# malani86/unet-DC-segmentation

Hardware: AMD Instinct MI355X
Metric: images/sec fwd+bwd, 512x512x1 U-Net-DC, bs=8/GPU (higher is better)
Workload: dtype bf16

## Files before the change

quantify_droplets_batch.py:

```python
#!/usr/bin/env python3
import argparse
import dataclasses
from pathlib import Path

import numpy as np
import pandas as pd
import torch
from PIL import Image

from models.model_2 import UNetDC
from unet_dc_segmentation_amd.droplets import DropletOptions, Droplets, resize_mask_like_reference
from utils import intensity_window as iw
from utils.data_loader import resize_image, rolling_ball_correction_rgb

DEVICE = "cuda" if torch.cuda.is_available() else "cpu"
IMG_SIZE = 512


def load_model(ckpt, dtype="f32"):
    m = UNetDC(in_channels=3, out_channels=1)
    m.load_state_dict(torch.load(ckpt, map_location=DEVICE, weights_only=True))
    m.set_compute_dtype(dtype)
    return m.to(DEVICE).eval()

# ... 763 lines not shown
        raise SystemExit("--boundary measures against annotated masks: it needs --gt_dir")
    from utils.droplet_boundary import DEFAULT_TOLS, check_radius, check_tols
    try:
        R = check_radius(args.boundary)
        tols = DEFAULT_TOLS if args.boundary_tol is None else [int(v) for v in args.boundary_tol.split(",") if v.strip()]
        tols = check_tols([t for t in tols if args.boundary_tol is not None or t <= R], R)
    except ValueError as e:
        raise SystemExit(f"--boundary R / --boundary_tol: {e}")
    return {"R": R, "tols": tols, "records": []}


def confidence_options(args):
    if args.confidence is None:
        if args.confidence_maps:
            raise SystemExit("--confidence_maps needs --confidence")
        return None
    from utils.droplet_confidence import check_band
    try:
        band = check_band(args.confidence)
    except ValueError as e:
        raise SystemExit(f"--confidence BAND: {e}")
    return {"band": band, "maps": bool(args.confidence_maps), "rows": []}


def spatial_options(args, images):
    if args.spatial_stats is None:
        if args.spatial_window_dir:
            raise SystemExit("--spatial_window_dir belongs to --spatial_stats")
        return None
    from utils.spatial_stats import check_sims
    try:
        sims = check_sims(args.spatial_sims)
    except ValueError as e:
        raise SystemExit(f"--spatial_sims S: {e}")
    if not 0 <= args.spatial_seed < 2 ** 32:
        raise SystemExit("--spatial_seed must be in 0..2^32 - 1")
    files = None
    if args.spatial_window_dir:
        files = find_gt_files(images, args.spatial_window_dir, "--spatial_window_dir", "window")
    return {"R": args.spatial_stats, "S": sims, "seed": args.spatial_seed, "files": files, "table": [], "rows": []}


def tile_options(args):
    if args.tile is None:
        if args.tile_overlap is not None:
            raise SystemExit("--tile_overlap needs --tile")
        return None
    from utils.tiling import check_tile
    try:
        T, O = check_tile(args.tile, 64 if args.tile_overlap is None else args.tile_overlap)
    except ValueError as e:
        raise SystemExit(f"--tile / --tile_overlap: {e}")
    if args.batch < 1:
        raise SystemExit("--tile: --batch is the number of tiles per forward, at least 1")
    return {"T": T, "O": O}


def tta_options(args):
    if args.tta is None:
        return None
    from utils.tta import TTA_SIZES
    if args.tta not in TTA_SIZES:
        raise SystemExit(f"--tta N: N must be one of {', '.join(map(str, TTA_SIZES))}, not {args.tta}")
    if args.batch < 1:
        raise SystemExit("--tta: --batch is the number of items per forward, at least 1")
    return None if args.tta == 1 else {"N": args.tta, "batch": args.batch}


def main(argv=None):
    parser = build_parser()
    args = parser.parse_args(argv)
    if args.gt_dir and args.gt_polygons:
        parser.error("--gt_polygons and --gt_dir are two sources of the same annotation: give one")
    if args.diff_maps is not None and not (args.gt_dir or args.gt_polygons):
        parser.error("--diff_maps compares against annotated masks: it needs --gt_dir")
    if args.diff_maps is not None and args.diff_maps < 1:
        parser.error("--diff_maps MIN_AREA: MIN_AREA is a number of pixels, at least 1")
    in_dir, out_dir = Path(args.img_dir), Path(args.out_dir)
    try:
        spec = iw.spec_from_flags(args.intensity_window, args.intensity_levels, args.page)
    except ValueError as e:
        parser.error(str(e))
    intensity = None if spec is None else {"spec": spec, "records": []}
    iw.clip_warner.done = False
    from utils.droplet_split import half_pixels
    try:
        split_depth = half_pixels(args.split_depth) / 2.0
    except ValueError:
        raise SystemExit("--split_depth must be a non-negative multiple of 0.5")
    if not args.split_touching:
        split_depth = None
    clean = clean_options(args)
    sweep = sweep_options(args)
    tile = tile_options(args)
    tta = tta_options(args)
    boundary = boundary_options(args)
    confidence = confidence_options(args)
    hull = None
    if args.droplet_hull is not None:
        from utils.droplet_hull import check_solidity
        try:
            hull = check_solidity(args.droplet_hull)
        except ValueError as e:
            raise SystemExit(f"--droplet_hull S: {e}")
    images = sorted(p for p in in_dir.iterdir() if p.suffix.lower() in IMAGE_SUFFIXES)
    gt = None
    if args.gt_dir:
        gt = {"files": find_gt_files(images, args.gt_dir), "min_area": args.gt_min_area, "labels": args.gt_labels}
    elif args.gt_polygons:
        gt = {"polygons": find_gt_polygons(images, args.gt_polygons), "min_area": 1, "labels": True, "features": 0, "dropped": 0}
    spatial = spatial_options(args, images)
    mask_dir = out_dir / "predicted_masks"
    overlay_dir = out_dir / "overlays" if args.save_overlays else None
    out_dir.mkdir(parents=True, exist_ok=True)
    mask_dir.mkdir(exist_ok=True)
    if overlay_dir:
        overlay_dir.mkdir(exist_ok=True)
    density = None
    if args.density_maps:
        if not 1 <= args.nb_layers <= 255 or not 0 < args.density_kernel or int(4 * args.density_kernel / 6 + 0.5) > 128:
            raise SystemExit("--nb_layers must be in 1..255 and --density_kernel in 1..192")
        density = {"nb_layers": args.nb_layers, "kernel": args.density_kernel}
    diff = None
    if args.diff_maps is not None:
        diff = {"min_area": args.diff_maps, "map_dir": out_dir / "difference_maps", "overlay_dir": out_dir / "diff_overlays",
                "tables": [], "rows": []}
        diff["map_dir"].mkdir(exist_ok=True)
        diff["overlay_dir"].mkdir(exist_ok=True)
    outlines = None
    if args.outlines:
        outlines = {"dir": out_dir / "outlines", "images": [], "jobs": []}
        outlines["dir"].mkdir(exist_ok=True)
    model = load_model(args.ckpt_path, args.dtype)
    import os
    from collections import deque
    from concurrent.futures import ThreadPoolExecutor
    nthreads = max(1, min(8, (os.cpu_count() or 2) // 2))
    with ThreadPoolExecutor(nthreads) as dec_pool, ThreadPoolExecutor(nthreads) as wr_pool:
        run = Run(thresh=args.prob_thresh, min_area=args.min_area, px_per_um=args.px_per_micron,
                  background_radius=args.background_radius, batch_size=args.batch, split_depth=split_depth,
                  shape=args.droplet_shape, clean=clean, sweep=sweep, tile=tile, tta=tta, density=density, gt=gt, out_dir=out_dir,
                  mask_dir=mask_dir, overlay_dir=overlay_dir, writers=(wr_pool, deque(), 4 * max(1, args.batch)),
                  neighbors=args.neighbors, boundary=boundary, confidence=confidence, hull=hull, diff=diff,
                  spatial=spatial, outlines=outlines, intensity=intensity)
        ahead = deque()
        it = iter(images)

        def refill():
            while len(ahead) < 2 * args.batch:
                nxt = next(it, None)
                if nxt is None:
                    return
                ahead.append((nxt, dec_pool.submit(decode_image, nxt, intensity),
                              None if gt is None else dec_pool.submit(decode_gt_polygons, gt["polygons"][str(nxt)]) if "polygons" in gt
                              else dec_pool.submit(decode_gt, gt["files"][str(nxt)], gt["labels"]),
                              None if spatial is None or spatial["files"] is None
                              else dec_pool.submit(decode_gt, spatial["files"][str(nxt)], False)))

        refill()
        batch = Batch()
        while ahead:
            img, fut, gt_fut, win_fut = ahead.popleft()
            refill()
            im = fut.result()
            if intensity is not None:
                im = window_image(run, img, *im)
            batch.meta.append((str(img), tuple(int(v) for v in im.shape[:2])))
            if run.shape:
                from utils.density import rgb_to_gray
                batch.grays.append(rgb_to_gray(_host(im)))
            if gt is not None:
                batch.gt_items.append(gt_fut.result())
            if win_fut is not None:
                batch.windows.append(win_fut.result())
            if tile is not None:
                probs, rgb = predict_tiled_image(model, _host(im), run)
                batch.rgbs.append(rgb)
                finish_batch(run, batch, probs)
                batch = Batch()
                continue
            t, _, *rgb = preprocess(img, args.background_radius, im, keep_rgb=run.keep_rgb)
            batch.tensors.append(t)
            batch.rgbs += rgb
            if len(batch.tensors) == args.batch:
                run_batch(run, batch, model)
                batch = Batch()
        if batch.tensors:
            run_batch(run, batch, model)
        for f in run.writers[1]:
            f.result()
    if intensity is not None:
        rows = [iw.record_row(name, mode, spec, n, {k: _host(v) for k, v in rec.items()}) for name, mode, n, rec in intensity["records"]]
        pd.DataFrame(rows).to_csv(out_dir / "intensity_per_image.csv", index=False)
    if density is not None:
        pd.DataFrame(run.density_rows).to_csv(out_dir / "density_per_image.csv", index=False)
    if gt is not None:
        from utils.droplet_match import pooled_row, summary_row
        tables = [t for t in run.gt_tables if len(t)] or run.gt_tables[:1]
        pd.concat(tables, ignore_index=True).to_csv(out_dir / "gt_droplets.csv", index=False) if tables else None
        rows = [summary_row(name, ints) for name, ints in run.gt_images] + [pooled_row([ints for _, ints in run.gt_images])]
        pd.DataFrame(rows).to_csv(out_dir / "match_per_image.csv", index=False)
        if "polygons" in gt:
            print(f"--gt_polygons: {gt['dropped']} of {gt['features']} features own no pixel centre and were dropped")
    if boundary is not None:
        from utils import droplet_boundary as db
        recs = boundary["records"]
        rows = [db.summary_row(name, h, d, boundary["R"], boundary["tols"]) for name, h, d in recs]
        rows.append(db.pooled_row([(h, d) for _, h, d in recs], boundary["R"], boundary["tols"]))
        pd.DataFrame(rows, columns=db.column_names(boundary["tols"])).to_csv(out_dir / "boundary_per_image.csv", index=False)
    if confidence is not None:
        from utils.droplet_confidence import IMAGE_COLUMNS
        pd.DataFrame(confidence["rows"], columns=("filename",) + IMAGE_COLUMNS).to_csv(out_dir / "confidence_per_image.csv", index=False)
    if diff is not None:
        from utils import difference_map as dmap
        tables = [t for t in diff["tables"] if len(t)] or diff["tables"][:1]
        pd.concat(tables, ignore_index=True).to_csv(out_dir / "diff_regions.csv", index=False) if tables else None
        pd.DataFrame(diff["rows"], columns=("filename",) + dmap.IMAGE_COLUMNS).to_csv(out_dir / "diff_regions_per_image.csv", index=False)
    if spatial is not None:
        from utils import spatial_stats as ss
        pd.DataFrame(spatial["table"], columns=ss.table_columns(run.px_per_um)).to_csv(out_dir / "spatial_stats.csv", index=False)
        pd.DataFrame(spatial["rows"], columns=ss.IMAGE_COLUMNS).to_csv(out_dir / "spatial_per_image.csv", index=False)
    if outlines is not None:
        import json
        anns = [a for job in outlines["jobs"] for a in job.result()]
        for i, a in enumerate(anns, start=1):
            a["id"] = i
        with open(out_dir / "outlines_coco.json", "w") as f:
            f.write(json.dumps({"images": outlines["images"], "annotations": anns, "categories": [{"id": 1, "name": "droplet"}]},
                               separators=(",", ":")))
    if clean is not None:
        pd.DataFrame(clean["rows"]).to_csv(out_dir / "mask_clean_per_image.csv", index=False)
    if run.neighbors is not None and run.contact_tables:
        pd.concat(run.contact_tables, ignore_index=True).to_csv(out_dir / "droplet_contacts.csv", index=False)
    if sweep is not None and sweep["hist"] is not None:
        from utils.threshold_sweep import summary_line, table_rows
        hist = sweep["hist"]
        if torch.is_tensor(hist):
            from unet_dc_segmentation_amd.evaluate import sweep_result
            hist = sweep_result(hist)
        pd.DataFrame(table_rows(hist)).to_csv(out_dir / "threshold_sweep.csv", index=False)
        print(summary_line(hist))
        if sweep["objects"]:
            from utils.droplet_match import pooled_row
            rows = []
            for t in sweep["objects"]:
                row = pooled_row(sweep["object_images"][t])
                row.pop("filename")
                rows.append({"threshold": t, **row})
            pd.DataFrame(rows).to_csv(out_dir / "threshold_sweep_objects.csv", index=False)
    summary_df = pd.DataFrame(run.rows)
    summary_df.to_csv(out_dir / "summary_per_image.csv", index=False)
    props = [d for d in run.tables if not d.empty]
    if props:
        combined = pd.concat(props, ignore_index=True)
        combined.to_csv(out_dir / "all_droplets.csv", index=False)
        if not args.skip_excel:
            try:
                import xlsxwriter
                with pd.ExcelWriter(out_dir / "all_droplets.xlsx", engine="xlsxwriter") as xw:
                    combined.to_excel(xw, index=False, sheet_name="droplets")
                    summary_df.to_excel(xw, index=False, sheet_name="per_image")
            except (ImportError, AttributeError):
                combined.to_csv(out_dir / "all_droplets_noexcel.csv", index=False)
                print("Skipped Excel file (xlsxwriter not available); wrote all_droplets_noexcel.csv")
        size_col = "eq_diam_micron" if "eq_diam_micron" in combined.columns else "equivalent_diameter"
        stats = combined[size_col].describe()[["mean", "50%", "std"]].rename({"50%": "median"})
        stats.to_csv(out_dir / "droplet_size_stats.csv")
        if not args.skip_histogram:
            import matplotlib
            matplotlib.use("Agg")
            import matplotlib.pyplot as plt
            plt.figure(figsize=(6, 4))
            plt.hist(combined[size_col], bins=40)
# ... 13 lines not shown
```

unet_dc_segmentation_amd/build.py:

```python
from __future__ import annotations

import os
import shutil
import subprocess
import sys

HERE = os.path.dirname(os.path.abspath(__file__))
CSRC = os.path.join(HERE, "csrc")
SOURCES = ["abi.hip", "igemm_conv.hip", "igemm_dma.hip", "igemm_dma16.hip", "igemm_halo.hip", "igemm_lattice.hip", "wgrad.hip", "wgrad_dma.hip", "wgrad_fused.hip", "wgrad_rect.hip", "convt_wgrad.hip", "first_conv.hip", "first_conv_mfma.hip", "partials.hip", "batchnorm.hip", "head.hip", "pack.hip", "loss.hip", "optim.hip", "ccl.hip", "split.hip", "shape.hip", "confidence.hip", "hull.hip", "outlines.hip", "polyfill.hip", "match.hip", "neighbors.hip", "spatial.hip", "boundary.hip", "diffmap.hip", "clean.hip", "sweep.hip", "tile.hip", "tta.hip", "preprocess.hip", "window.hip", "augment.hip", "crop.hip", "density.hip", "border.hip"]
HEADERS = ["common.h", "kernels.h", "workspace.h", "partials.h", "bn_bwd_terms.h", "ccl_uf.h", "pair_table.h", "wave_ops.h", "lds_dma.h", "wgrad_frag.h", "igemm_epilogue.h", "igemm_epilogue16.h", "gather_index.h", "linear_u8.h", "hash32.h", os.path.join("..", "..", "include", "unetdc_hip.h")]
OUT = os.path.join(HERE, "libunetdc_hip.so")


def _hipcc():
    for cand in (shutil.which("hipcc"), "/opt/rocm/bin/hipcc"):
        if cand and os.path.exists(cand):
            return cand
    raise RuntimeError("hipcc not found (ROCm toolchain required to build the gfx950 kernels)")


def needs_build():
    if not os.path.exists(OUT):
        return True
    t = os.path.getmtime(OUT)
    deps = [os.path.join(CSRC, f) for f in SOURCES + HEADERS]
    return any(os.path.getmtime(d) > t for d in deps)


FLAGS = ["--offload-arch=gfx950", "-O3", "-std=c++17", "-fPIC", "-Wall", "-Wno-unused-function", "-fno-slp-vectorize"]
OBJ_DIR = os.path.join(CSRC, "_obj")


def _includes(path, seen=None):
    import re
    seen = set() if seen is None else seen
    for m in re.finditer(r'^\s*#include\s+"([^"]+)"', open(path).read(), re.M):
        q = os.path.normpath(os.path.join(os.path.dirname(path), m.group(1)))
        if q not in seen and os.path.exists(q):
            seen.add(q)
            _includes(q, seen)
    return seen


def _object_key(src):
    import hashlib
    h = hashlib.sha256(" ".join(FLAGS).encode())
    for q in [src] + sorted(_includes(src)):
        h.update(open(q, "rb").read())
    return h.hexdigest()[:16]


def build(force=False, verbose=True):
    if not force and not needs_build():
        return OUT
    from concurrent.futures import ThreadPoolExecutor
    os.makedirs(OBJ_DIR, exist_ok=True)
    hipcc = _hipcc()

    def one(f):
        src = os.path.join(CSRC, f)
        obj = os.path.join(OBJ_DIR, f"{os.path.splitext(f)[0]}.{_object_key(src)}.o")
        if force or not os.path.exists(obj):
            for old in os.listdir(OBJ_DIR):
                if old.startswith(os.path.splitext(f)[0] + "."):
                    os.unlink(os.path.join(OBJ_DIR, old))
            cmd = [hipcc, *FLAGS, "-c", src, "-o", obj]
            if verbose:
                print("[unetdc build]", " ".join(cmd), flush=True)
            r = subprocess.run(cmd, capture_output=True, text=True)
            if r.returncode != 0:
                sys.stderr.write(r.stdout + r.stderr)
                raise RuntimeError(f"hipcc failed on {f}")
        return obj

    with ThreadPoolExecutor(max_workers=min(8, os.cpu_count() or 1)) as ex:
        objs = list(ex.map(one, SOURCES))
    cmd = [hipcc, "--offload-arch=gfx950", "-shared", "-fPIC", *objs, "-o", OUT]
    r = subprocess.run(cmd, capture_output=True, text=True)
    if r.returncode != 0:
        sys.stderr.write(r.stdout + r.stderr)
        raise RuntimeError("hipcc failed linking libunetdc_hip.so")
    return OUT


def _objdump():
    for cand in (shutil.which("llvm-objdump"), "/opt/rocm/lib/llvm/bin/llvm-objdump"):
        if cand and os.path.exists(cand):
            return cand
    raise RuntimeError("llvm-objdump not found")


def device_code_objects(so_path=OUT):
# ... 44 lines not shown
```

unet_dc_segmentation_amd/csrc/igemm_conv.hip:

```cpp
#include <stdlib.h>

#include <stdio.h>

#include "kernels.h"

namespace unetdc {

template <typename T> struct Mma;
template <> struct Mma<bf16_t> {
  __device__ static __forceinline__ void run(f32x16& acc, const u32x4& a, const u32x4& b) {
    acc = __builtin_amdgcn_mfma_f32_32x32x16_bf16(__builtin_bit_cast(bf16x8, a), __builtin_bit_cast(bf16x8, b),
                                                  acc, 0, 0, 0);
  }
};
template <> struct Mma<float> {
  __device__ static __forceinline__ void run(f32x16& acc, const u32x4& a, const u32x4& b) {
#pragma unroll
    for (int s = 0; s < 4; ++s) {
      const unsigned int ua = a[s], ub = b[s];
      acc = __builtin_amdgcn_mfma_f32_32x32x2f32(bits_f32(ua), bits_f32(ub), acc, 0, 0, 0);
    }
  }
};

// ... 180 lines not shown
        store_pair<T>(og + (long)m * p.ldo + col, v0, v1);
        if (p.mode == MODE_STATS) {
          const float t0 = round_through<T>(v0), t1 = round_through<T>(v1);
          s0 += t0; q0 = fmaf(t0, t0, q0);
          s1 += t1; q1 = fmaf(t1, t1, q1);
        }
      }
    }
  }
  if (p.mode == MODE_STATS) {
    s0 += __shfl_xor(s0, 32, 64); q0 += __shfl_xor(q0, 32, 64);
    s1 += __shfl_xor(s1, 32, 64); q1 += __shfl_xor(q1, 32, 64);
    float* red = reinterpret_cast<float*>(smem);
    if (h == 0) {
      red[(wave * 4 + 0) * 32 + r] = s0;
      red[(wave * 4 + 1) * 32 + r] = q0;
      red[(wave * 4 + 2) * 32 + r] = s1;
      red[(wave * 4 + 3) * 32 + r] = q1;
    }
    __syncthreads();
    if (tid < BN) {
      const int wn2 = tid >> 6, c2 = tid & 63, r2 = c2 >> 1, e = c2 & 1;
      float su = 0.f, sq = 0.f;
#pragma unroll
      for (int w2 = 0; w2 < WM; ++w2) {
        su += red[((w2 * WN + wn2) * 4 + e * 2 + 0) * 32 + r2];
        sq += red[((w2 * WN + wn2) * 4 + e * 2 + 1) * 32 + r2];
      }
      p.stats[((long)mblk * 2 + 0) * p.Cout + n0 + tid] = su;
      p.stats[((long)mblk * 2 + 1) * p.Cout + n0 + tid] = sq;
    }
  }
}

int igemm_mblocks(long M, int Cout) { (void)Cout; return ceil_div(M, 256); }

template <typename T, int WM, int WN>
static int launch_cfg(IgemmParams& p, hipStream_t stream) {
  constexpr int BM = 64 * WM, BN = 64 * WN;
  constexpr int LDS = 2 * (BM + BN) * 128;
  if (const int rc_ = ensure_dynamic_lds(reinterpret_cast<const void*>(&igemm_conv_kernel<T, WM, WN>), LDS, "igemm_conv_kernel")) return rc_;
  p.mblocks = ceil_div(p.M, BM);
  p.nblocks = p.Cout / BN;
  const long nwg = (long)p.mblocks * p.nblocks;
  hipLaunchKernelGGL((igemm_conv_kernel<T, WM, WN>), dim3((unsigned)nwg), dim3(256), LDS, stream, p);
  char nm[96];
  snprintf(nm, sizeof(nm), "igemm_conv_kernel<%s, %d, %d>", sizeof(T) == 2 ? "__bf16" : "float", WM, WN);
  note_kernel(nm);
  return check_launch("igemm_conv_kernel");
}

IgemmPlan plan_igemm(const IgemmParams& p, int dtype) {
  IgemmPlan pl{};
  const bool lattice = igemm_lattice_supported(p, dtype);
  if (p.in_scale) {
    if (lattice && p.mode == MODE_STATS && (p.Cout % 128 == 0 || p.Cin <= 256)) {
      pl.route = IGEMM_LATTICE;
      pl.writes_act = p.Cout % 128 == 0 && (long)p.M * p.Cin * 2 < (1L << 32);
    }
    return pl;
  }
  if (lattice) {
    pl.route = IGEMM_LATTICE;
    return pl;
  }
  if (igemm_halo_supported(p, dtype)) {
    pl.route = IGEMM_HALO;
    return pl;
  }
  const long es = dtype == UNETDC_BF16 ? 2 : 4;
  const long HoWo = (long)p.Ho * p.Wo;
  const long xbytes = (p.M / HoWo) * p.Hi * p.Wi * p.ldx * es;
  const long wbytes = (long)p.ntaps * p.Cout * p.Cin * es;
  const long opix = p.mode == MODE_SHUFFLE ? 4L * p.M : (long)p.M;
  const long obytes = opix * p.ldo * es, ybytes = p.mode == MODE_BNBWD ? (long)p.M * p.bn_ldy * es : 0;
  if (!(xbytes < (1L << 31) && wbytes < (1L << 31) && obytes < (1L << 32) && ybytes < (1L << 32) && p.M % HoWo == 0)) {
    pl.route = IGEMM_FIRSTGEN;
    pl.cfg = (p.Cout % 128 == 0) && p.mode != MODE_STATS;
    return pl;
  }
  const long blocks_a = (long)((p.M + 255) / 256) * (p.Cout / 256);
  const bool use_a = p.Cout % 256 == 0 && p.M >= 256 * 64 && blocks_a >= 200;
  const bool use_b = !use_a && p.Cout % 128 == 0;
  pl.route = IGEMM_DMA;
  pl.cfg = use_a ? 1 : (use_b ? 2 : 3);
  if (dtype == UNETDC_BF16 && p.M % 16 == 0 && !(p.mode == MODE_SHUFFLE && p.Wo % 16 != 0)) {
    pl.route = IGEMM_DMA16;
    const long blocks_b = (long)((p.M + 255) / 256) * (p.Cout / 128);
    if (pl.cfg == 2 && p.mode == MODE_SHUFFLE && p.Cout % 256 == 0 && blocks_a >= 200) pl.cfg = 1;
    else if (pl.cfg == 2 && blocks_b >= 100 && blocks_b < 200) pl.cfg = 3;
  }
  return pl;
}

int launch_igemm(IgemmParams& p, int dtype, hipStream_t stream) {
  const int esz = dtype == UNETDC_BF16 ? 2 : 4;
  const int ke = 128 / esz;
  UNETDC_REQUIRE(dtype == UNETDC_F32 || dtype == UNETDC_BF16, "igemm: bad dtype %d", dtype);
  UNETDC_REQUIRE(p.x && p.w && p.out, "igemm: null tensor pointer");
  UNETDC_REQUIRE(p.M > 0 && p.Cin > 0 && p.Cout > 0, "igemm: empty problem");
  UNETDC_REQUIRE(p.Cin % ke == 0, "igemm: Cin=%d must be a multiple of %d for this dtype", p.Cin, ke);
  UNETDC_REQUIRE(p.Cout % 64 == 0, "igemm: Cout=%d must be a multiple of 64", p.Cout);
  UNETDC_REQUIRE(p.ldx % (16 / esz) == 0 && p.ldo % (16 / esz) == 0, "igemm: ld not 16-byte aligned");
  UNETDC_REQUIRE(((uintptr_t)p.x % 16 == 0) && ((uintptr_t)p.w % 16 == 0) && ((uintptr_t)p.out % 16 == 0),
                 "igemm: pointers must be 16-byte aligned");
  UNETDC_REQUIRE(p.ntaps >= 1 && p.ntaps <= 9, "igemm: ntaps out of range");
  UNETDC_REQUIRE((long)p.M < (1L << 31) - 512, "igemm: too many pixels");
  if (p.mode == MODE_SHUFFLE) UNETDC_REQUIRE(p.shuf_c % 64 == 0, "igemm: convT channels must be a multiple of 64");
  if (p.mode == MODE_STATS) UNETDC_REQUIRE(p.stats != nullptr, "igemm: stats buffer missing");
  if (p.mode == MODE_AFFINE_RELU) UNETDC_REQUIRE(p.scale && p.shift, "igemm: scale/shift missing");
  if (p.mode == MODE_BNBWD)
    UNETDC_REQUIRE(p.stats && p.bn_y && p.scale && p.shift && p.bn_mean && p.bn_rstd, "igemm: BN-backward inputs missing");
  {
    const long howo = (long)p.Ho * p.Wo;
    const bool p2 = (p.Wo & (p.Wo - 1)) == 0 && (howo & (howo - 1)) == 0;
    p.wo_shift = p2 ? __builtin_ctz((unsigned)p.Wo) : -1;
    p.howo_shift = p2 ? __builtin_ctzl((unsigned long)howo) : -1;
  }
  const IgemmPlan pl = plan_igemm(p, dtype);
  switch (pl.route) {
    case IGEMM_LATTICE: return launch_igemm_lattice(p, stream);
    case IGEMM_HALO: return launch_igemm_halo(p, dtype, stream);
    case IGEMM_DMA: return launch_igemm_dma(p, pl.cfg, dtype, stream);
    case IGEMM_DMA16: return launch_igemm_dma16(p, pl.cfg, stream);
    case IGEMM_FIRSTGEN:
      if (p.mode == MODE_BNBWD) {
        set_error("igemm: the first-generation kernel has no fused BatchNorm-backward sums");
        return UNETDC_EUNSUPPORTED;
      }
      if (dtype == UNETDC_BF16) return pl.cfg ? launch_cfg<bf16_t, 2, 2>(p, stream) : launch_cfg<bf16_t, 4, 1>(p, stream);
      return pl.cfg ? launch_cfg<float, 2, 2>(p, stream) : launch_cfg<float, 4, 1>(p, stream);
  }
  set_error("igemm: input normalisation asked for a shape / configuration the lattice kernel does not take");
  return UNETDC_EUNSUPPORTED;
}

}
```

unet_dc_segmentation_amd/csrc/kernels.h:

```cpp
#pragma once
#include <algorithm>
#include <type_traits>

#include "common.h"
#include "workspace.h"
#include "../../include/unetdc_hip.h"

namespace unetdc {

enum { MODE_STORE = 0, MODE_STATS = 1, MODE_AFFINE_RELU = 2, MODE_SHUFFLE = 3, MODE_BNBWD = 4 };
#define UNETDC_EUNSUPPORTED (-4)

struct IgemmParams {
  const void* x;
  const void* w;
  void* out;
  const float* bias;
  const float* scale;
  const float* shift;
  float* stats;
  const void* bn_y;
  const float* bn_mean;
  const float* bn_rstd;
  int bn_ldy;
  int M, Ho, Wo, Hi, Wi, Cin, Cout, ldx, ldo, ntaps, stride, mode, shuf_c;
  int mblocks, nblocks;
  int wo_shift, howo_shift;
  int quad_bpr, quad_bpi;
  const float* in_scale;
  const float* in_shift;
  void* act_out;
  int ld_act;
  int offy[9];
  int offx[9];
};
enum IgemmRoute {
  IGEMM_UNSUPPORTED = 0,
  IGEMM_LATTICE,
  IGEMM_HALO,
  IGEMM_DMA,
  IGEMM_DMA16,
  IGEMM_FIRSTGEN,
};
struct IgemmPlan {
  int route;
  int cfg;
  bool writes_act;
};
IgemmPlan plan_igemm(const IgemmParams& p, int dtype);
int launch_igemm(IgemmParams& p, int dtype, hipStream_t stream);
int igemm_mblocks(long M, int Cout);
bool igemm_lattice_supported(const IgemmParams& p, int dtype);
bool igemm_halo_supported(const IgemmParams& p, int dtype);
int launch_igemm_lattice(IgemmParams& p, hipStream_t stream);
int launch_igemm_halo(IgemmParams& p, int dtype, hipStream_t stream);
int launch_igemm_dma(IgemmParams& p, int cfg, int dtype, hipStream_t stream);
int launch_igemm_dma16(IgemmParams& p, int cfg, hipStream_t stream);

struct WgradParams {
  const void* a;
  const void* b;
  float* part;
  int N, H, W, Hb, Wb, CI, CJ, lda, ldb, ntaps, stride;
  int P;
  int chunk;
  int ksplit, itiles, jtiles;
  int adv_y, adv_x;
  int offy[9];
  int offx[9];
  const float* in_scale;
  const float* in_shift;
};
enum WgradRoute {
  WGRAD_UNSUPPORTED = 0,
  WGRAD_CONVT,
  WGRAD_RECT,
  WGRAD_FUSED,
  WGRAD_DMA,
  WGRAD_LEGACY,
};
struct WgradFusedPlan {
  bool supported;
  bool paired;
  bool bnin;
  int pf;
  int ysplit, rows_per_unit, imgs_per_unit, half_lds;
  int threads, nwg;
  int lds, lds_attr;
  int units;
  long workspace;
};
struct WgradPlan {
  int route;
  WgradFusedPlan fused;
  int ksplit;
  int chunk, tw, step;
  int steps_per_half;
  long workspace;
};
WgradPlan plan_wgrad(const WgradParams& p, int dtype);
long wgrad_workspace_bound(int N, int H, int W, int CI, int CJ, int ntaps, int dtype);
int launch_wgrad(WgradParams& p, float* out, void* workspace, long workspace_bytes, int dtype, hipStream_t stream);
bool convt_wgrad_split(int N, int H, int W, int CI, int CJ, int& ksplit, int& steps_per_half);
int launch_convt_wgrad_fused(const WgradParams& w, const WgradPlan& pl, hipStream_t stream);
int wgrad_rect_units(int N, int H, int W, int CI, int CJ, int d);
int launch_wgrad_rect(const WgradParams& w, const WgradPlan& pl, float* out, hipStream_t stream);
WgradFusedPlan plan_wgrad_fused(const WgradParams& w, int dtype);
long wgrad_fused_workspace_bytes(int N, int H, int W, int CI, int CJ, int dtype);
int launch_wgrad_fused(const WgradParams& w, const WgradFusedPlan& pl, int dtype, hipStream_t stream);
int wgrad_dma_tile(int CI, int CJ);
int wgrad_dma_pixel_step(int dtype, int tw);
int launch_wgrad_dma_kernel(WgradParams& p, int tw, int dtype, hipStream_t stream);

struct FirstParams {
  const float* x;
  const float* w;
  const float* bias;
  const float* scale;
  const float* shift;
  void* y;
  float* stats;
  int N, H, W, Cin, Cout, ldy, dil;
};
struct FirstWgradParams {
  const float* x;
  const void* dy;
  float* part;
  int N, H, W, Cin, Cout, lddy, dil;
  const void* bn_y; int bn_ldy;
  const float* bn_scale; const float* bn_shift; const float* bn_mean; const float* bn_rstd; const float* bn_k;
};
struct FirstPlan {
  bool mfma;
  int fwd_blocks;
  bool wgrad_mfma;
  int wgrad_blocks;
  int rows_blocks;
  long workspace;
};
FirstPlan plan_first(long P, int Cin, int Cout);
// ... 258 lines not shown
```

utils/intensity_window.py:

```python
from __future__ import annotations

import dataclasses
from decimal import Decimal, InvalidOperation

import numpy as np

PPM = 10 ** 6
MAX_RANKS = 8
MAX_PLANES = 256
DEFAULT_WINDOW = "0.1,99.9"
DEEP_MODES = ("I;16", "I;16L", "I;16B", "I;16N", "I", "F")
FLAG_HELP = "--intensity_window"


@dataclasses.dataclass(frozen=True)
class WindowSpec:
    plo: int
    phi: int
    levels: tuple | None = None
    page: int | str = 0

    @property
    def ppm(self):
        return (0, self.plo, PPM // 2, self.phi, PPM)
# ... 134 lines not shown
    if not 1 <= len(ppm) <= MAX_RANKS or any(p < 0 or p > PPM for p in ppm):
        raise ValueError(f"1..{MAX_RANKS} ranks in 0..{PPM} parts per million are expected")
    return ppm


def ranks_numpy(arr, ppm):
    arr = np.asarray(arr)
    if arr.dtype != np.uint16 or arr.ndim != 3 or not 1 <= arr.shape[2] <= 4 or arr.shape[0] * arr.shape[1] < 1:
        raise ValueError("ranks: uint16 [h, w, c] with c in 1..4 is expected")
    ppm = check_ppm(ppm)
    h, w, c = arr.shape
    n = h * w
    out = np.zeros((3, c, len(ppm)), np.int32)
    for ch in range(c):
        s = np.sort(arr[:, :, ch], axis=None)
        for j, p in enumerate(ppm):
            v = s[rank_index(p, n) - 1]
            lo, hi = np.searchsorted(s, v, "left"), np.searchsorted(s, v, "right")
            out[:, ch, j] = (int(v), int(lo), int(hi - lo))
    return out[0], out[1], out[2]


def window_numpy(arr, levels, dc=None):
    arr = np.asarray(arr)
    h, w, c = arr.shape
    dc = c if dc is None else int(dc)
    if arr.dtype != np.uint16 or not (dc == c or (dc == 3 and c == 1)):
        raise ValueError("window: uint16 [h, w, c] and dc == c, or dc == 3 with c == 1")
    levels = np.clip(np.asarray(levels, np.int64).reshape(c, 2), 0, 65535)
    out = np.zeros((h, w, c), np.uint8)
    for ch in range(c):
        lo, hi = int(levels[ch, 0]), int(levels[ch, 1])
        d = hi - lo
        if d > 0:
            t = np.clip(arr[:, :, ch].astype(np.int64), lo, hi) - lo
            out[:, :, ch] = (510 * t + d) // (2 * d)
    return np.repeat(out, 3, axis=2) if dc != c else out


def out_channels(c):
    return 3 if c == 1 else c


def levels_of(spec, value):
    c = value.shape[0]
    if spec.levels is not None:
        return np.tile(np.asarray(spec.levels, np.int32), (c, 1))
    return np.ascontiguousarray(value[:, [1, 3]]).astype(np.int32)


def deep_to_u8_numpy(arr, spec):
    value, below, equal = ranks_numpy(arr, spec.ppm)
    levels = levels_of(spec, value)
    return window_numpy(arr, levels, out_channels(arr.shape[2])), {"ranks": np.stack((value, below, equal)), "levels": levels}


def record_row(filename, mode, spec, n, record):
    value, below, equal = (np.asarray(record["ranks"][i], np.int64) for i in range(3))
    levels = np.asarray(record["levels"], np.int64)
    row = {"filename": filename, "mode": mode, "page": spec.page, "pixels": int(n), "p_lo_ppm": spec.plo, "p_hi_ppm": spec.phi}
    for ch in range(value.shape[0]):
        k = f"ch{ch}_"
        row[k + "min"], row[k + "p_lo"], row[k + "median"], row[k + "p_hi"], row[k + "max"] = (int(v) for v in value[ch])
        row[k + "lo"], row[k + "hi"] = int(levels[ch, 0]), int(levels[ch, 1])
        if spec.levels is None:
            row[k + "clipped_low_frac"] = int(below[ch, 1]) / n
            row[k + "clipped_high_frac"] = (n - int(below[ch, 3]) - int(equal[ch, 3])) / n
        else:
            row[k + "clipped_low_frac"] = row[k + "clipped_high_frac"] = ""
        row[k + "saturated"] = int(equal[ch, 4]) if int(value[ch, 4]) == 65535 else 0
    return row


def clip_warning(path, mode):
    return (f"warning: {path} is a deep image (mode {mode}); without {FLAG_HELP} its values were clipped at 255 "
            f"(further deep images are not reported)")


class ClipWarner:

    def __init__(self):
        import threading
        self.done = False
        self.lock = threading.Lock()

    def __call__(self, path, mode):
        if self.done or not is_deep(mode):
            return
        with self.lock:
            first, self.done = not self.done, True
        if first:
            print(clip_warning(path, mode), flush=True)


clip_warner = ClipWarner()


def decode_rgb_clipped(path):
    from PIL import Image
    with Image.open(path) as im:
        clip_warner(path, im.mode)
        return np.array(im.convert("RGB"))
```

Baseline: 743.6.

## Add streaming kernels for transposed-conv forward and data-gradient

```diff
diff --git a/quantify_droplets_batch.py b/quantify_droplets_batch.py
--- a/quantify_droplets_batch.py
+++ b/quantify_droplets_batch.py
@@ -869,7 +869,7 @@
     except ValueError as e:
         parser.error(str(e))
     intensity = None if spec is None else {"spec": spec, "records": []}
-    iw.clip_warner.done = False
+    iw.clip_warner.arm(in_order=True)
     from utils.droplet_split import half_pixels
     try:
         split_depth = half_pixels(args.split_depth) / 2.0
@@ -950,6 +950,7 @@
             img, fut, gt_fut, win_fut = ahead.popleft()
             refill()
             im = fut.result()
+            iw.clip_warner.consumed(img)
             if intensity is not None:
                 im = window_image(run, img, *im)
             batch.meta.append((str(img), tuple(int(v) for v in im.shape[:2])))
@@ -976,6 +977,7 @@
             run_batch(run, batch, model)
         for f in run.writers[1]:
             f.result()
+    iw.clip_warner.arm()
     if intensity is not None:
         rows = [iw.record_row(name, mode, spec, n, {k: _host(v) for k, v in rec.items()}) for name, mode, n, rec in intensity["records"]]
         pd.DataFrame(rows).to_csv(out_dir / "intensity_per_image.csv", index=False)
diff --git a/unet_dc_segmentation_amd/build.py b/unet_dc_segmentation_amd/build.py
--- a/unet_dc_segmentation_amd/build.py
+++ b/unet_dc_segmentation_amd/build.py
@@ -7,7 +7,7 @@
 
 HERE = os.path.dirname(os.path.abspath(__file__))
 CSRC = os.path.join(HERE, "csrc")
-SOURCES = ["abi.hip", "igemm_conv.hip", "igemm_dma.hip", "igemm_dma16.hip", "igemm_halo.hip", "igemm_lattice.hip", "wgrad.hip", "wgrad_dma.hip", "wgrad_fused.hip", "wgrad_rect.hip", "convt_wgrad.hip", "first_conv.hip", "first_conv_mfma.hip", "partials.hip", "batchnorm.hip", "head.hip", "pack.hip", "loss.hip", "optim.hip", "ccl.hip", "split.hip", "shape.hip", "confidence.hip", "hull.hip", "outlines.hip", "polyfill.hip", "match.hip", "neighbors.hip", "spatial.hip", "boundary.hip", "diffmap.hip", "clean.hip", "sweep.hip", "tile.hip", "tta.hip", "preprocess.hip", "window.hip", "augment.hip", "crop.hip", "density.hip", "border.hip"]
+SOURCES = ["abi.hip", "igemm_conv.hip", "igemm_dma.hip", "igemm_dma16.hip", "igemm_halo.hip", "igemm_lattice.hip", "wgrad.hip", "wgrad_dma.hip", "wgrad_fused.hip", "wgrad_rect.hip", "convt_wgrad.hip", "convt_stream.hip", "first_conv.hip", "first_conv_mfma.hip", "partials.hip", "batchnorm.hip", "head.hip", "pack.hip", "loss.hip", "optim.hip", "ccl.hip", "split.hip", "shape.hip", "confidence.hip", "hull.hip", "outlines.hip", "polyfill.hip", "match.hip", "neighbors.hip", "spatial.hip", "boundary.hip", "diffmap.hip", "clean.hip", "sweep.hip", "tile.hip", "tta.hip", "preprocess.hip", "window.hip", "augment.hip", "crop.hip", "density.hip", "border.hip"]
 HEADERS = ["common.h", "kernels.h", "workspace.h", "partials.h", "bn_bwd_terms.h", "ccl_uf.h", "pair_table.h", "wave_ops.h", "lds_dma.h", "wgrad_frag.h", "igemm_epilogue.h", "igemm_epilogue16.h", "gather_index.h", "linear_u8.h", "hash32.h", os.path.join("..", "..", "include", "unetdc_hip.h")]
 OUT = os.path.join(HERE, "libunetdc_hip.so")
 
diff --git a/unet_dc_segmentation_amd/csrc/convt_stream.hip b/unet_dc_segmentation_amd/csrc/convt_stream.hip
--- /dev/null
+++ b/unet_dc_segmentation_amd/csrc/convt_stream.hip
@@ -0,0 +1,326 @@
+#include <stdio.h>
+
+#include "igemm_epilogue16.h"
+#include "kernels.h"
+#include "lds_dma.h"
+
+namespace unetdc {
+
+constexpr int CS_T = 32;
+constexpr int CS_NS = 4;
+constexpr int CS_CUS = 256;
+
+template <int CIN, int COUT>
+__global__ __launch_bounds__(512) void convt_stream_fwd_kernel(const IgemmParams p) {
+#if defined(__HIP_DEVICE_COMPILE__)
+  constexpr int KG = CIN / 32;
+  constexpr int WN = 4 * COUT / 64;
+  constexpr int WM = 8 / WN;
+  constexpr int TMT = CS_T / 16 / WM;
+  constexpr int STAGE = CS_T * CIN * 2;
+  constexpr int PER = STAGE / 1024 / 8;
+  constexpr int NST = TMT * 4;
+  constexpr int STEADY = NST + (CS_NS - 2) * (PER + NST);
+  static_assert(WN * WM == 8 && TMT >= 1 && PER >= 1 && STEADY <= 63, "tile / wave mismatch");
+  extern __shared__ __attribute__((aligned(16))) unsigned char smem[];
+
+  const int tid = threadIdx.x, lane = tid & 63;
+  const int wave = __builtin_amdgcn_readfirstlane(tid >> 6);
+  const int wm = wave / WN, wn = wave % WN;
+  const int c16 = lane & 15, rb = lane >> 4;
+  const int G = gridDim.x;
+  const int first = blockIdx.x;
+  const int nitems = p.M / CS_T;
+  const int mine = first < nitems ? (nitems - first + G - 1) / G : 0;
+  const unsigned lds_base = lds_addr_of(smem);
+  const __amdgpu_buffer_rsrc_t xr =
+      __builtin_amdgcn_make_buffer_rsrc(const_cast<void*>(p.x), 0, (unsigned)((long)p.M * p.ldx * 2), 0x00020000);
+
+  unsigned asrc[PER];
+#pragma unroll
+  for (int j = 0; j < PER; ++j) {
+    const int q = wave + 8 * j;
+    const int row = (q & 3) * 8 + (lane >> 3);
+    const int c = (lane & 7) ^ ((row >> 1) & 7);
+    asrc[j] = (unsigned)(row * p.ldx * 2 + (q >> 2) * 128 + c * 16);
+  }
+  auto issue = [&](int it, int stage) {
+    const unsigned soff = (unsigned)__builtin_amdgcn_readfirstlane((first + it * G) * CS_T * p.ldx * 2);
+    const unsigned sbase = lds_base + (unsigned)__builtin_amdgcn_readfirstlane(stage) * STAGE;
+#pragma unroll
+    for (int j = 0; j < PER; ++j) lds_dma16(xr, sbase + (wave + 8 * j) * 1024, asrc[j], soff);
+  };
+#pragma unroll
+  for (int k = 0; k < CS_NS - 1; ++k)
+    if (k < mine) issue(k, k);
+
+  u32x4 wreg[KG][4];
+  {
+    const unsigned char* wb = reinterpret_cast<const unsigned char*>(p.w);
+#pragma unroll
+    for (int g = 0; g < KG; ++g)
+#pragma unroll
+      for (int j = 0; j < 4; ++j)
+        wreg[g][j] = ld16(wb + ((long)(wn * 64 + 4 * c16 + j) * CIN + g * 32 + rb * 8) * 2);
+  }
+  const int ab = (wn * 64) / COUT, co = (wn * 64) % COUT + 4 * c16;
+  float k1[4];
+#pragma unroll
+  for (int k = 0; k < 4; ++k) k1[k] = p.bias ? p.bias[co + k] : 0.f;
+  const __amdgpu_buffer_rsrc_t orr = whole_buffer(p.out);
+  const unsigned ldob = (unsigned)(p.ldo * 2);
+  const unsigned lane_off = (unsigned)(2 * (wm * TMT * 16 + 4 * rb)) * ldob + (unsigned)(co * 2);
+
+  const int swz = (c16 >> 1) & 7;
+  int a_rd[2];
+#pragma unroll
+  for (int g = 0; g < 2; ++g) a_rd[g] = (wm * TMT * 16 + c16) * 128 + (((4 * g + rb) ^ swz) << 4);
+
+  int cur = 0, fill = CS_NS - 1;
+  for (int s = 0; s < mine; ++s) {
+    if (s + CS_NS - 2 >= mine) wait_vmcnt<0>();
+    else if (s < CS_NS - 1) wait_vmcnt<(CS_NS - 2) * PER>();
+    else wait_vmcnt<STEADY>();
+    raw_barrier();
+    if (s + CS_NS - 1 < mine) issue(s + CS_NS - 1, fill);
+    const unsigned char* base = smem + cur * STAGE;
+    f32x4 acc[TMT][4];
+#pragma unroll
+    for (int i = 0; i < TMT; ++i)
+#pragma unroll
+      for (int j = 0; j < 4; ++j)
+#pragma unroll
+        for (int e = 0; e < 4; ++e) acc[i][j][e] = 0.f;
+#pragma unroll
+    for (int g = 0; g < KG; ++g)
+#pragma unroll
+      for (int i = 0; i < TMT; ++i) {
+        const u32x4 fa = ld16(base + (g >> 1) * (CS_T * 128) + a_rd[g & 1] + i * 16 * 128);
+#pragma unroll
+        for (int j = 0; j < 4; ++j)
+          acc[i][j] = __builtin_amdgcn_mfma_f32_16x16x32_bf16(__builtin_bit_cast(bf16x8, fa), __builtin_bit_cast(bf16x8, wreg[g][j]),
+                                                              acc[i][j], 0, 0, 0);
+      }
+    const int m0 = (first + s * G) * CS_T;
+    const int R = m0 / p.Wo, x0 = m0 - R * p.Wo;
+    const unsigned item_off =
+        (unsigned)__builtin_amdgcn_readfirstlane((int)(((unsigned)(2 * R + (ab >> 1)) * (unsigned)(2 * p.Wo) + (unsigned)(2 * x0 + (ab & 1))) * ldob));
+#pragma unroll
+    for (int i = 0; i < TMT; ++i)
+#pragma unroll
+      for (int v = 0; v < 4; ++v) {
+        const u32x2 pk = pack4_bf16(acc[i][0][v] + k1[0], acc[i][1][v] + k1[1], acc[i][2][v] + k1[2], acc[i][3][v] + k1[3]);
+        __builtin_amdgcn_raw_buffer_store_b64(pk, orr, lane_off + (unsigned)(i * 32) * ldob, item_off + (unsigned)(2 * v) * ldob, 0);
+      }
+    cur = cur + 1 == CS_NS ? 0 : cur + 1;
+    fill = fill + 1 == CS_NS ? 0 : fill + 1;
+  }
+#endif
+}
+
+constexpr int CD_T = 64, CD_NS = 3, CD_CI = 128, CD_CO = 64, CD_BM = 256;
+
+template <bool BN>
+__global__ __launch_bounds__(512) void convt_stream_dgrad_kernel(const IgemmParams p) {
+#if defined(__HIP_DEVICE_COMPILE__)
+  constexpr int KG = 4 * CD_CO / 32;
+  constexpr int SUB = CD_T * 128;
+  constexpr int NSUB = 4 + (BN ? 2 : 0);
+  constexpr int STAGE = NSUB * SUB;
+  constexpr int PER = NSUB;
+  constexpr int NST = 4;
+  constexpr int STEADY = (CD_NS - 1) * NST + (CD_NS - 2) * PER;
+  extern __shared__ __attribute__((aligned(16))) unsigned char smem[];
+
+  const int tid = threadIdx.x, lane = tid & 63;
+  const int wave = __builtin_amdgcn_readfirstlane(tid >> 6);
+  const int wm = wave >> 1, wn = wave & 1;
+  const int c16 = lane & 15, rb = lane >> 4;
+  const int G = gridDim.x;
+  const int first = blockIdx.x;
+  const int nblocks = p.M / CD_BM;
+  const int mine = first < nblocks ? 4 * ((nblocks - first + G - 1) / G) : 0;
+  const unsigned lds_base = lds_addr_of(smem);
+  const __amdgpu_buffer_rsrc_t xr =
+      __builtin_amdgcn_make_buffer_rsrc(const_cast<void*>(p.x), 0, (unsigned)(4L * p.M * p.ldx * 2), 0x00020000);
+  const __amdgpu_buffer_rsrc_t yr =
+      __builtin_amdgcn_make_buffer_rsrc(const_cast<void*>(BN ? p.bn_y : p.x), 0, BN ? (unsigned)((long)p.M * p.bn_ldy * 2) : 0u, 0x00020000);
+
+  const int ssub = lane >> 3;
+  const int sc = (lane & 7) ^ (((wave * 8 + ssub) >> 1) & 7);
+  const unsigned dsrc0 = (unsigned)(2 * ssub * p.ldx * 2 + sc * 16);
+  const unsigned ysrc0 = BN ? (unsigned)(ssub * p.bn_ldy * 2 + sc * 16) : 0u;
+  auto issue = [&](int it, int stage) {
+    const int p0 = (first + (it >> 2) * G) * CD_BM + (wave >> 1) * 64 + (it & 3) * 16 + (wave & 1) * 8;
+    const int R = p0 / p.Wo, x0 = p0 - R * p.Wo;
+    const unsigned sbase = lds_base + (unsigned)__builtin_amdgcn_readfirstlane(stage) * STAGE + wave * 1024;
+#pragma unroll
+    for (int a = 0; a < 2; ++a) {
+      const unsigned soff = (unsigned)__builtin_amdgcn_readfirstlane((int)(((unsigned)(2 * R + a) * (unsigned)(2 * p.Wo) + (unsigned)(2 * x0)) * (unsigned)(p.ldx * 2)));
+      lds_dma16(xr, sbase + (2 * a) * SUB, dsrc0, soff);
+      lds_dma16(xr, sbase + (2 * a + 1) * SUB, dsrc0 + (unsigned)(p.ldx * 2), soff);
+    }
+    if (BN) {
+      const unsigned soff = (unsigned)__builtin_amdgcn_readfirstlane((int)((unsigned)p0 * (unsigned)(p.bn_ldy * 2)));
+      lds_dma16(yr, sbase + 4 * SUB, ysrc0, soff);
+      lds_dma16(yr, sbase + 5 * SUB, ysrc0 + 128u, soff);
+    }
+  };
+#pragma unroll
+  for (int k = 0; k < CD_NS - 1; ++k)
+    if (k < mine) issue(k, k);
+
+  u32x4 wreg[KG][4];
+  {
+    const unsigned char* wb = reinterpret_cast<const unsigned char*>(p.w);
+#pragma unroll
+    for (int g = 0; g < KG; ++g)
+#pragma unroll
+      for (int j = 0; j < 4; ++j)
+        wreg[g][j] = ld16(wb + (((long)(g >> 1) * CD_CI + wn * 64 + 4 * c16 + j) * CD_CO + (g & 1) * 32 + rb * 8) * 2);
+  }
+  const int col = wn * 64 + 4 * c16;
+  const Epi16Consts kc = epi16_consts<BN ? MODE_BNBWD : MODE_STORE>(p, col);
+  float s4[4] = {0.f, 0.f, 0.f, 0.f}, q4[4] = {0.f, 0.f, 0.f, 0.f};
+  const __amdgpu_buffer_rsrc_t orr = whole_buffer(p.out);
+  const unsigned ldob = (unsigned)(p.ldo * 2);
+  const unsigned lane_off = (unsigned)(wm * 64 + 4 * rb) * ldob + (unsigned)(col * 2);
+  float* red = reinterpret_cast<float*>(smem + CD_NS * STAGE);
+
+  const int swz = (c16 >> 1) & 7;
+  int a_rd[2];
+#pragma unroll
+  for (int g = 0; g < 2; ++g) a_rd[g] = (wm * 16 + c16) * 128 + (((4 * g + rb) ^ swz) << 4);
+  int y_rd[4];
+#pragma unroll
+  for (int v = 0; v < 4; ++v) {
+    const int row = wm * 16 + 4 * rb + v;
+    y_rd[v] = (4 + wn) * SUB + row * 128 + ((((c16 >> 1) ^ (row >> 1)) & 7) << 4) + (c16 & 1) * 8;
+  }
+
+  int cur = 0, fill = CD_NS - 1;
+  for (int s = 0; s < mine; ++s) {
+    if (s + CD_NS - 2 >= mine) wait_vmcnt<0>();
+    else if (s < CD_NS - 1) wait_vmcnt<(CD_NS - 2) * PER>();
+    else wait_vmcnt<STEADY>();
+    raw_barrier();
+    if (s + CD_NS - 1 < mine) issue(s + CD_NS - 1, fill);
+    const unsigned char* base = smem + cur * STAGE;
+    f32x4 acc[4];
+#pragma unroll
+    for (int j = 0; j < 4; ++j)
+#pragma unroll
+      for (int e = 0; e < 4; ++e) acc[j][e] = 0.f;
+#pragma unroll
+    for (int g = 0; g < KG; ++g) {
+      const u32x4 fa = ld16(base + (g >> 1) * SUB + a_rd[g & 1]);
+#pragma unroll
+      for (int j = 0; j < 4; ++j)
+        acc[j] = __builtin_amdgcn_mfma_f32_16x16x32_bf16(__builtin_bit_cast(bf16x8, fa), __builtin_bit_cast(bf16x8, wreg[g][j]), acc[j], 0, 0, 0);
+    }
+    const int blk = first + (s >> 2) * G;
+    const unsigned item_off = (unsigned)__builtin_amdgcn_readfirstlane((int)((unsigned)(blk * CD_BM + (s & 3) * 16) * ldob));
+#pragma unroll
+    for (int v = 0; v < 4; ++v) {
+      const u32x2 pk = pack4_bf16(acc[0][v], acc[1][v], acc[2][v], acc[3][v]);
+      __builtin_amdgcn_raw_buffer_store_b64(pk, orr, lane_off, item_off + (unsigned)v * ldob, 0);
+      if (BN) {
+        const u32x2 yraw = *reinterpret_cast<const u32x2*>(base + y_rd[v]);
+        float t[4], y[4];
+        unpack4_bf16(pk, t);
+        unpack4_bf16(yraw, y);
+#pragma unroll
+        for (int k = 0; k < 4; ++k) {
+          const float gk = fmaf(y[k], kc.k0[k], kc.k1[k]) > 0.f ? t[k] : 0.f;
+          s4[k] += gk;
+          q4[k] = fmaf(gk, (y[k] - kc.mu[k]) * kc.rs[k], q4[k]);
+        }
+      }
+    }
+    if (BN && (s & 3) == 3) {
+#pragma unroll
+      for (int k = 0; k < 4; ++k) {
+        s4[k] += __shfl_xor(s4[k], 16, 64); q4[k] += __shfl_xor(q4[k], 16, 64);
+        s4[k] += __shfl_xor(s4[k], 32, 64); q4[k] += __shfl_xor(q4[k], 32, 64);
+      }
+      if (rb == 0) {
+#pragma unroll
+        for (int k = 0; k < 4; ++k) {
+          red[((wave * 4 + k) * 2 + 0) * 16 + c16] = s4[k];
+          red[((wave * 4 + k) * 2 + 1) * 16 + c16] = q4[k];
+        }
+      }
+      asm volatile("s_waitcnt lgkmcnt(0)" ::: "memory");
+      raw_barrier();
+      if (tid < CD_CI) {
+        const int wn2 = tid >> 6, cc = tid & 63, c2 = cc >> 2, k = cc & 3;
+        float su = 0.f, sq = 0.f;
+#pragma unroll
+        for (int w2 = 0; w2 < 4; ++w2) {
+          su += red[(((w2 * 2 + wn2) * 4 + k) * 2 + 0) * 16 + c2];
+          sq += red[(((w2 * 2 + wn2) * 4 + k) * 2 + 1) * 16 + c2];
+        }
+        p.stats[((long)blk * 3 + 0) * CD_CI + tid] = su;
+        p.stats[((long)blk * 3 + 1) * CD_CI + tid] = sq;
+        p.stats[((long)blk * 3 + 2) * CD_CI + tid] = 0.f;
+      }
+#pragma unroll
+      for (int k = 0; k < 4; ++k) { s4[k] = 0.f; q4[k] = 0.f; }
+    }
+    cur = cur + 1 == CD_NS ? 0 : cur + 1;
+    fill = fill + 1 == CD_NS ? 0 : fill + 1;
+  }
+#endif
+}
+
+bool convt_stream_fwd_supported(const IgemmParams& p, int dtype) {
+  if (dtype != UNETDC_BF16 || p.mode != MODE_SHUFFLE || p.ntaps != 1 || p.stride != 1) return false;
+  if (!((p.Cin == 128 && p.shuf_c == 64) || (p.Cin == 256 && p.shuf_c == 128)) || p.Cout != 4 * p.shuf_c) return false;
+  if (p.Wo % CS_T != 0 || p.Hi != p.Ho || p.Wi != p.Wo || p.M % ((long)p.Ho * p.Wo) != 0) return false;
+  if (p.M < 32768) return false;
+  return (long)p.M * p.ldx * 2 < (1L << 31) && 4L * p.M * p.ldo * 2 < (1L << 32);
+}
+
+template <int CIN, int COUT>
+static int launch_convt_stream_cfg(const IgemmParams& p, int wgs_per_cu, hipStream_t stream) {
+  constexpr int LDS = CS_NS * CS_T * CIN * 2;
+  if (const int rc_ = ensure_dynamic_lds(reinterpret_cast<const void*>(&convt_stream_fwd_kernel<CIN, COUT>), LDS, "convt_stream_kernel")) return rc_;
+  const long items = p.M / CS_T, fit = (long)CS_CUS * wgs_per_cu;
+  const long grid = items < fit ? items : fit;
+  hipLaunchKernelGGL((convt_stream_fwd_kernel<CIN, COUT>), dim3((unsigned)grid), dim3(512), LDS, stream, p);
+  char nm[96];
+  snprintf(nm, sizeof(nm), "convt_stream_kernel<fwd, %d, %d>", CIN, COUT);
+  note_kernel(nm);
+  return check_launch("convt_stream_kernel");
+}
+
+int launch_convt_stream_fwd(IgemmParams& p, hipStream_t stream) {
+  if (p.Cin == 128) return launch_convt_stream_cfg<128, 64>(p, 2, stream);
+  return launch_convt_stream_cfg<256, 128>(p, 1, stream);
+}
+
+bool convt_stream_dgrad_supported(const IgemmParams& p, int dtype) {
+  if (dtype != UNETDC_BF16 || (p.mode != MODE_STORE && p.mode != MODE_BNBWD) || p.ntaps != 4 || p.stride != 2) return false;
+  for (int t = 0; t < 4; ++t)
+    if (p.offy[t] != (t >> 1) || p.offx[t] != (t & 1)) return false;
+  if (p.Cin != CD_CO || p.Cout != CD_CI || p.Hi != 2 * p.Ho || p.Wi != 2 * p.Wo) return false;
+  if (p.Wo % 32 != 0 || p.M % CD_BM != 0 || p.M % ((long)p.Ho * p.Wo) != 0 || p.M < 32768) return false;
+  const long ybytes = p.mode == MODE_BNBWD ? (long)p.M * p.bn_ldy * 2 : 0;
+  return 4L * p.M * p.ldx * 2 < (1L << 31) && (long)p.M * p.ldo * 2 < (1L << 32) && ybytes < (1L << 32);
+}
+
+int launch_convt_stream_dgrad(IgemmParams& p, hipStream_t stream) {
+  const bool bn = p.mode == MODE_BNBWD;
+  const int LDS = CD_NS * (bn ? 6 : 4) * CD_T * 128 + (bn ? 8 * 128 * 4 : 0);
+  const void* fn = bn ? reinterpret_cast<const void*>(&convt_stream_dgrad_kernel<true>) : reinterpret_cast<const void*>(&convt_stream_dgrad_kernel<false>);
+  if (const int rc_ = ensure_dynamic_lds(fn, LDS, "convt_stream_kernel")) return rc_;
+  p.mblocks = p.M / CD_BM;
+  p.nblocks = 1;
+  const int grid = p.mblocks < CS_CUS ? p.mblocks : CS_CUS;
+  if (bn) hipLaunchKernelGGL(convt_stream_dgrad_kernel<true>, dim3((unsigned)grid), dim3(512), LDS, stream, p);
+  else hipLaunchKernelGGL(convt_stream_dgrad_kernel<false>, dim3((unsigned)grid), dim3(512), LDS, stream, p);
+  note_kernel(bn ? "convt_stream_kernel<dgrad_bnstats, 128, 64>" : "convt_stream_kernel<dgrad, 128, 64>");
+  return check_launch("convt_stream_kernel");
+}
+
+}
diff --git a/unet_dc_segmentation_amd/csrc/igemm_conv.hip b/unet_dc_segmentation_amd/csrc/igemm_conv.hip
--- a/unet_dc_segmentation_amd/csrc/igemm_conv.hip
+++ b/unet_dc_segmentation_amd/csrc/igemm_conv.hip
@@ -286,6 +286,10 @@
   const long blocks_a = (long)((p.M + 255) / 256) * (p.Cout / 256);
   const bool use_a = p.Cout % 256 == 0 && p.M >= 256 * 64 && blocks_a >= 200;
   const bool use_b = !use_a && p.Cout % 128 == 0;
+  if (convt_stream_fwd_supported(p, dtype) || convt_stream_dgrad_supported(p, dtype)) {
+    pl.route = IGEMM_CONVT_STREAM;
+    return pl;
+  }
   pl.route = IGEMM_DMA;
   pl.cfg = use_a ? 1 : (use_b ? 2 : 3);
   if (dtype == UNETDC_BF16 && p.M % 16 == 0 && !(p.mode == MODE_SHUFFLE && p.Wo % 16 != 0)) {
@@ -327,6 +331,7 @@
     case IGEMM_HALO: return launch_igemm_halo(p, dtype, stream);
     case IGEMM_DMA: return launch_igemm_dma(p, pl.cfg, dtype, stream);
     case IGEMM_DMA16: return launch_igemm_dma16(p, pl.cfg, stream);
+    case IGEMM_CONVT_STREAM: return p.mode == MODE_SHUFFLE ? launch_convt_stream_fwd(p, stream) : launch_convt_stream_dgrad(p, stream);
     case IGEMM_FIRSTGEN:
       if (p.mode == MODE_BNBWD) {
         set_error("igemm: the first-generation kernel has no fused BatchNorm-backward sums");
diff --git a/unet_dc_segmentation_amd/csrc/kernels.h b/unet_dc_segmentation_amd/csrc/kernels.h
--- a/unet_dc_segmentation_amd/csrc/kernels.h
+++ b/unet_dc_segmentation_amd/csrc/kernels.h
@@ -40,6 +40,7 @@
   IGEMM_HALO,
   IGEMM_DMA,
   IGEMM_DMA16,
+  IGEMM_CONVT_STREAM,
   IGEMM_FIRSTGEN,
 };
 struct IgemmPlan {
@@ -56,6 +57,10 @@
 int launch_igemm_halo(IgemmParams& p, int dtype, hipStream_t stream);
 int launch_igemm_dma(IgemmParams& p, int cfg, int dtype, hipStream_t stream);
 int launch_igemm_dma16(IgemmParams& p, int cfg, hipStream_t stream);
+bool convt_stream_fwd_supported(const IgemmParams& p, int dtype);
+int launch_convt_stream_fwd(IgemmParams& p, hipStream_t stream);
+bool convt_stream_dgrad_supported(const IgemmParams& p, int dtype);
+int launch_convt_stream_dgrad(IgemmParams& p, hipStream_t stream);
 
 struct WgradParams {
   const void* a;
diff --git a/utils/intensity_window.py b/utils/intensity_window.py
--- a/utils/intensity_window.py
+++ b/utils/intensity_window.py
@@ -240,14 +240,30 @@
     def __init__(self):
         import threading
         self.done = False
+        self.noted = None
         self.lock = threading.Lock()
+
+    def arm(self, in_order=False):
+        self.done, self.noted = False, {} if in_order else None
 
     def __call__(self, path, mode):
         if self.done or not is_deep(mode):
             return
         with self.lock:
+            if self.noted is not None:
+                self.noted[str(path)] = mode
+                return
             first, self.done = not self.done, True
         if first:
+            print(clip_warning(path, mode), flush=True)
+
+    def consumed(self, path):
+        if self.done or self.noted is None:
+            return
+        with self.lock:
+            mode = self.noted.pop(str(path), None)
+        if mode is not None:
+            self.done = True
             print(clip_warning(path, mode), flush=True)
 
 
```

After: 748.3 (median of 6 runs). No clear change (+0.6%).
